# agustinus/emqx

Hardware: AMD Instinct MI355X
Metric: publishes matched/sec (node) at 1M wildcard subs; p99 batch match latency (higher is better)
Workload: dtype u32; 1 GPU; C2: 1M wildcard filters depth<=7, 10M-publish batch per GPU; filters=1000000, publishes_per_gpu=10000000, mode=replicated, parallelism=replicated trie x1, batches split per GPU, batches_in_flight=1

## Files before the change

emqx_amd/csrc/tm_kernels.hip:

```cpp
#include <algorithm>
#include <cstddef>
#include <cstdlib>
#include "tm_internal.hpp"

namespace etm {

constexpr int TILE = 64;
constexpr int WCAP = 512;
#ifndef TM_WPE384
#define TM_WPE384 4
#endif

constexpr uint32_t M_LVL_SHIFT = 6;
constexpr uint32_t M_LVL_MASK = 0xF;
constexpr uint32_t M_PLUS = 1u << 10;
constexpr uint32_t M_SKIPE = 1u << 11;
constexpr uint32_t M_DSTART = 1u << 12;
static_assert(FAST_MAX_DEPTH <= (int)M_LVL_MASK, "level field too narrow");
constexpr uint32_t M_DISP_SHIFT = 13;
constexpr uint32_t M_DISP_MASK = 0x3F;
static_assert(MAX_PROBE_DISP <= M_DISP_MASK, "the displacement field holds every bounded probe run");
constexpr uint32_t Q_FOUND = ~((1u << LSIG_BITS) - 1u);
constexpr uint32_t Q_TAIL = 0xFFFFFFFFu;

__device__ __forceinline__ uint32_t dig_L(uint32_t c) { return (0x4432u >> (4 * c)) & 0xF; }
__device__ __forceinline__ uint32_t dig_H(uint32_t c) { return (0x2223u >> (4 * c)) & 0xF; }
__device__ __forceinline__ uint32_t dig_P(uint32_t c) { return (0x3344u >> (4 * c)) & 0xF; }

__device__ __forceinline__ int key_shift(uint32_t level) { return 61 - 3 * (int)level; }

__device__ __forceinline__ uint64_t put_digit(uint64_t key, uint32_t level, uint32_t d) {
    return level <= FAST_MAX_DEPTH ? (key | ((uint64_t)d << key_shift(level))) : key;
}

__device__ __forceinline__ uint32_t prefix_count(uint64_t mask) {
    return __builtin_amdgcn_mbcnt_hi((uint32_t)(mask >> 32), __builtin_amdgcn_mbcnt_lo((uint32_t)mask, 0u));
}

template <bool CK>
__device__ __forceinline__ uint64_t ck(uint64_t i, uint64_t bound, uint32_t* dbg, uint32_t id) {
    if (CK && i >= bound) {
        if (dbg) {
            if (atomicCAS(&dbg[0], 0u, id) == 0u) { dbg[1] = (uint32_t)i; dbg[2] = (uint32_t)bound; }
            atomicAdd(&dbg[3], 1u);
        }
        return 0;
    }
    return i;
}
#define CK_(i, bound, id) ck<CK>((i), (bound), a.dbg, (id))

struct Node {
    uint32_t child;
    uint32_t term;
    uint32_t hterm;
    uint32_t flags;
};

#ifndef TM_PROBE_CPOL
#define TM_PROBE_CPOL 0
#endif
__device__ __forceinline__ uint4 ld_b128(__amdgpu_buffer_rsrc_t r, uint32_t off) {
    const auto v = __builtin_amdgcn_raw_buffer_load_b128(r, (int)off, 0, TM_PROBE_CPOL);
    return uint4{v[0], v[1], v[2], v[3]};
}

template <bool CK, bool BIG>
__device__ __forceinline__ bool probe(const MatchArgs& a, uint32_t parent, uint32_t word, Node& n) {
    uint32_t b = home_bucket(parent, word, a.nbuckets);
    const bool small = !BIG;
    const __amdgpu_buffer_rsrc_t rs = __builtin_amdgcn_make_buffer_rsrc(
        const_cast<Slot*>(a.slots), 0, BIG ? 0u : a.nslots * 16u, 0x00020000);
    for (uint32_t p = 0; p <= a.max_probe; ++p) {
        uint4 s0, s1, s2, s3;
        const uint64_t si = CK_((uint64_t)b * BUCKET, a.nslots, 1);
        if (small) {
            const uint32_t off = (uint32_t)si * 16u;
            s0 = ld_b128(rs, off); s1 = ld_b128(rs, off + 16); s2 = ld_b128(rs, off + 32); s3 = ld_b128(rs, off + 48);
        } else {
            const uint4* q = reinterpret_cast<const uint4*>(a.slots) + si;
            s0 = q[0]; s1 = q[1]; s2 = q[2]; s3 = q[3];
        }
        const bool m0 = (s0.x & ID_MASK) == parent && (s0.y & WID_MASK) == word;
        const bool m1 = (s1.x & ID_MASK) == parent && (s1.y & WID_MASK) == word;
        const bool m2 = (s2.x & ID_MASK) == parent && (s2.y & WID_MASK) == word;
        const bool m3 = (s3.x & ID_MASK) == parent && (s3.y & WID_MASK) == word;
        const uint32_t hz = m0 ? s0.z : m1 ? s1.z : m2 ? s2.z : s3.z;
        const uint32_t hw = m0 ? s0.w : m1 ? s1.w : m2 ? s2.w : s3.w;
        if (m0 | m1 | m2 | m3) {
            n.child = hz & ID_MASK;
            n.term = (hz & B_TOPIC) ? n.child : NONE;
            n.hterm = (hw & B_HTERM) ? (hw & ID_MASK) : NONE;
            n.flags = ((hz & B_PLUS) ? NF_PLUS : 0u) | ((hw & B_HASH) ? NF_HASH : 0u);
            return true;
        }
        if (s3.x == SLOT_EMPTY) return false;
        b = (b + 1 == a.nbuckets) ? 0 : b + 1;
    }
    return false;
}

struct Expand {
    uint32_t ne, np;
    uint32_t ef0, ef1;
    uint64_t ek0, ek1;
    uint32_t pf0, pf1;
    uint64_t pk0, pk1;
};

__device__ __forceinline__ void add_e(Expand& x, uint32_t fid, uint64_t key) {
    if (x.ne == 0) { x.ef0 = fid; x.ek0 = key; } else { x.ef1 = fid; x.ek1 = key; }
    x.ne++;
}
__device__ __forceinline__ void add_p(Expand& x, uint64_t key, uint32_t fl) {
    if (x.np == 0) { x.pk0 = key; x.pf0 = fl; } else { x.pk1 = key; x.pf1 = fl; }
    x.np++;
}

__device__ __forceinline__ void expand(const Node& s, uint32_t lc, uint32_t d, uint32_t flags,
                                       uint64_t key, uint32_t w_here, uint32_t w_prev, Expand& x) {
    x.ne = 0; x.np = 0;
    if (lc == d) {
        if (!(flags & M_SKIPE) && s.term != NONE) {
            uint64_t k = key;
            if ((w_prev >> WID_BITS) == C_EMPTY && lc - 1 <= FAST_MAX_DEPTH) {
                const int sp = key_shift(lc - 1);
                if (((k >> sp) & 7) == 4) k = (k & ~(7ull << sp)) | (1ull << sp);
            }
            add_e(x, s.term, k);
        }
        if (s.hterm != NONE) add_e(x, s.hterm, put_digit(key, lc, 2));
        return;
    }
    const uint32_t cls = w_here >> WID_BITS, id = w_here & WID_MASK;
    if (s.hterm != NONE) add_e(x, s.hterm, put_digit(key, lc, dig_H(cls)));
    if (id == W_HASH) {
        if (s.flags & NF_HASH) add_p(x, put_digit(key, lc, dig_L(cls)), (lc + 1 == d) ? M_SKIPE : 0u);
    } else if (id != W_UNKNOWN && id != W_PLUS) {
        add_p(x, put_digit(key, lc, dig_L(cls)), 0u);
    }
    if (s.flags & NF_PLUS) add_p(x, put_digit(key, lc, dig_P(cls)), M_PLUS);
}

__device__ __forceinline__ void expand_root(const RootRec& r, bool dollar, uint32_t d, uint32_t w0, Expand& x) {
    x.ne = 0; x.np = 0;
    const uint32_t cls = w0 >> WID_BITS, id = w0 & WID_MASK;
    if (!dollar && r.hterm != NONE) add_e(x, r.hterm, (uint64_t)dig_H(cls) << 61);
    if (id == W_HASH) {
        if (!dollar && (r.flags & NF_HASH)) add_p(x, (uint64_t)dig_L(cls) << 61, (d == 1) ? M_SKIPE : 0u);
    } else if (id != W_UNKNOWN && id != W_PLUS) {
        add_p(x, (uint64_t)dig_L(cls) << 61, dollar ? M_DSTART : 0u);
    }
    if (!dollar && (r.flags & NF_PLUS)) add_p(x, (uint64_t)dig_P(cls) << 61, M_PLUS);
}

template <int QC>
struct alignas(16) TileLds {
    static constexpr int QCAP = QC;
    uint4 q[QC];
    uint32_t words[WCAP];
    uint32_t toff[TILE];
    uint32_t depth[TILE];
    uint32_t cnt[TILE];
    uint32_t list[TILE];
    static constexpr uint32_t STAGE = (QC * 16 + WCAP * 4) / 8;
};

__device__ __forceinline__ uint4 q_pack(uint64_t key, uint32_t meta, uint32_t parent, uint32_t pw) {
    return uint4{(uint32_t)key | meta, (uint32_t)(key >> 32), parent, pw};
}

static_assert(offsetof(TileLds<512>, words) + sizeof(uint32_t) * WCAP == TileLds<512>::STAGE * 8,
              "staging area must be contiguous");
static_assert(offsetof(TileLds<384>, words) + sizeof(uint32_t) * WCAP == TileLds<384>::STAGE * 8,
              "staging area must be contiguous");

__device__ __forceinline__ uint32_t xor_lane32(uint32_t v, uint32_t j) {
    const uint32_t lane = threadIdx.x & 63;
    switch (j) {
    case 1: return (uint32_t)__builtin_amdgcn_mov_dpp((int)v, 0xB1, 0xF, 0xF, false);
    case 2: return (uint32_t)__builtin_amdgcn_mov_dpp((int)v, 0x4E, 0xF, 0xF, false);
    case 4: return (uint32_t)__builtin_amdgcn_mov_dpp(__builtin_amdgcn_mov_dpp((int)v, 0x141, 0xF, 0xF, false), 0x1B, 0xF,
                                                      0xF, false);
    case 8: return (uint32_t)__builtin_amdgcn_mov_dpp((int)v, 0x128, 0xF, 0xF, false);
    case 16: {
        const auto p = __builtin_amdgcn_permlane16_swap(v, v, false, false);
        return (lane & 16) ? p[0] : p[1];
    }
    default: {
        const auto p = __builtin_amdgcn_permlane32_swap(v, v, false, false);
        return (lane & 32) ? p[0] : p[1];
    }
    }
}

__device__ __forceinline__ unsigned long long xor_lane64(unsigned long long v, uint32_t j) {
    return ((unsigned long long)xor_lane32((uint32_t)(v >> 32), j) << 32) | xor_lane32((uint32_t)v, j);
}

__device__ __forceinline__ uint32_t tile_sum(uint32_t v) {
#pragma unroll
    for (uint32_t j = 1; j < 64; j <<= 1) v += xor_lane32(v, j);
    return __builtin_amdgcn_readfirstlane(v);
}

enum : int { PH_PROLOGUE = 0, PH_LOOP = 1, PH_READBACK = 2, PH_SORT = 3 };
struct PhaseClk {
#if TM_PHASE_CYCLES
    unsigned long long sum[PHASE_N] = {0, 0, 0, 0}, t0 = 0;
    __device__ __forceinline__ void start() { t0 = __builtin_readcyclecounter(); }
    __device__ __forceinline__ void lap(int p) {
        const unsigned long long now = __builtin_readcyclecounter();
        sum[p] += now - t0;
        t0 = now;
    }
#else
    __device__ __forceinline__ void start() {}
    __device__ __forceinline__ void lap(int) {}
#endif
};

__device__ __forceinline__ uint32_t xor_lane32_bc(uint32_t v, uint32_t j) {
    const int x = (int)v;
    switch (j) {
    case 1: return (uint32_t)__builtin_amdgcn_update_dpp(0, x, 0xB1, 0xF, 0xF, true);
    case 2: return (uint32_t)__builtin_amdgcn_update_dpp(0, x, 0x4E, 0xF, 0xF, true);
    case 4: return (uint32_t)__builtin_amdgcn_update_dpp(0, __builtin_amdgcn_update_dpp(0, x, 0x141, 0xF, 0xF, true),
                                                         0x1B, 0xF, 0xF, true);
    default: return (uint32_t)__builtin_amdgcn_update_dpp(0, x, 0x128, 0xF, 0xF, true);
    }
}

#ifndef TM_TAGGED_SORT
#define TM_TAGGED_SORT 1
#endif
constexpr uint64_t keep_lo_mask(uint32_t W, uint32_t kk, uint32_t j) {
    uint64_t m = 0;
    for (uint32_t l = 0; l < 64; ++l) {
        const uint32_t e = l & (W - 1);
        if (((e & j) == 0) == ((e & kk) == 0)) m |= 1ull << l;
    }
    return m;
}

template <uint32_t W, uint32_t KK, uint32_t J>
__device__ __forceinline__ uint32_t tag_stage(uint32_t k) {
    constexpr uint64_t M = keep_lo_mask(W, KK, J);
    uint32_t lo, hi;
    if constexpr (J >= 16) {
        const auto p = J == 16 ? __builtin_amdgcn_permlane16_swap(k, k, false, false)
                               : __builtin_amdgcn_permlane32_swap(k, k, false, false);
        lo = min(p[0], p[1]);
        hi = max(p[0], p[1]);
    } else {
        const uint32_t other = xor_lane32_bc(k, J);
        lo = min(k, other);
        hi = max(k, other);
    }
    return __builtin_amdgcn_inverse_ballot_w64(M) ? lo : hi;
}
template <uint32_t W, uint32_t KK, uint32_t J>
__device__ __forceinline__ uint32_t tag_merge(uint32_t k) {
    k = tag_stage<W, KK, J>(k);
    if constexpr (J > 1) k = tag_merge<W, KK, J / 2>(k);
    return k;
}
template <uint32_t W, uint32_t KK = 2>
__device__ __forceinline__ uint32_t tag_sort(uint32_t k) {
    k = tag_merge<W, KK, KK / 2>(k);
    if constexpr (KK < W) k = tag_sort<W, KK * 2>(k);
    return k;
}

template <bool CK, class LT>
__device__ __forceinline__ void sort_classes(const MatchArgs& a, LT& L, bool keep, uint32_t c, uint32_t pos,
                                             uint32_t dst, uint32_t free) {
    constexpr uint32_t STAGE = LT::STAGE;
    const uint32_t lane = threadIdx.x;
    const unsigned long long* stg = reinterpret_cast<const unsigned long long*>(L.q);
    if (keep && c == 1) a.sfids[CK_(dst, a.sfids_cap, 40)] = (uint32_t)(stg[CK_(pos, STAGE, 41)] & ~KEY_MASK);
#pragma unroll
    for (uint32_t W = 2; W <= 64; W <<= 1) {
        const bool mine = keep && c > W / 2 && c <= W;
        const uint64_t m = __ballot(mine);
        if (!m) continue;
        const uint32_t nrows = __popcll(m);
        if (mine) L.list[prefix_count(m)] = lane;
        __syncthreads();
        const uint32_t e = lane & (W - 1);
        const uint32_t STEP = 64 / W;
        for (uint32_t g = 0; g < nrows; g += STEP) {
            const uint32_t r = g + lane / W;
            const bool rv = r < nrows;
            const uint32_t owner = rv ? L.list[r] : 0u;
            const uint32_t cr = __shfl(c, owner, 64);
            const uint32_t pr = __shfl(pos, owner, 64);
            const uint32_t dr = __shfl(dst, owner, 64);
            if (TM_TAGGED_SORT && (W >> free) <= 1) {
                const uint32_t* stg32 = reinterpret_cast<const uint32_t*>(L.q);
                uint32_t k32 = 0xFFFFFFFFu;
                if (rv && e < cr) k32 = stg32[2 * CK_(pr + e, STAGE, 42) + 1] | e;
                switch (W) {
                case 2: k32 = tag_sort<2>(k32); break;
                case 4: k32 = tag_sort<4>(k32); break;
                case 8: k32 = tag_sort<8>(k32); break;
                case 16: k32 = tag_sort<16>(k32); break;
                case 32: k32 = tag_sort<32>(k32); break;
                default: k32 = tag_sort<64>(k32); break;
                }
                if (rv && e < cr)
                    a.sfids[CK_((uint64_t)dr + e, a.sfids_cap, 44)] =
                        stg32[2 * CK_(pr + (k32 & (W - 1)), STAGE, 43)] & (uint32_t)~KEY_MASK;
                continue;
            }
            unsigned long long key = ~0ull;
            if (rv && e < cr) key = stg[CK_(pr + e, STAGE, 42)];
#pragma unroll
            for (uint32_t kk = 2; kk <= W; kk <<= 1) {
#pragma unroll
                for (uint32_t j = kk >> 1; j > 0; j >>= 1) {
                    const unsigned long long other = xor_lane64(key, j);
                    const bool up = (e & kk) == 0;
                    const bool lower = (e & j) == 0;
                    const unsigned long long lo = key < other ? key : other;
                    const unsigned long long hi = key < other ? other : key;
                    key = (lower == up) ? lo : hi;
                }
            }
            if (rv && e < cr) a.sfids[CK_((uint64_t)dr + e, a.sfids_cap, 44)] = (uint32_t)(key & ~KEY_MASK);
        }
        __syncthreads();
    }
    {
        const bool mine = keep && c > 64;
        uint64_t m = __ballot(mine);
        while (m) {
            const uint32_t owner = (uint32_t)__builtin_ctzll(m);
            m &= m - 1;
            const uint32_t cr = __shfl(c, owner, 64);
            const uint32_t pr = __shfl(pos, owner, 64);
            const uint32_t dr = __shfl(dst, owner, 64);
            unsigned long long k0 = ~0ull, k1 = ~0ull;
            if (lane < cr) k0 = stg[CK_(pr + lane, STAGE, 45)];
            if (lane + 64 < cr) k1 = stg[CK_(pr + lane + 64, STAGE, 46)];
            uint32_t r0 = 0, r1 = 0;
            for (uint32_t j = 0; j < 64; ++j) {
                const unsigned long long kj = __shfl(k0, j, 64);
                r0 += kj < k0 ? 1u : 0u;
                r1 += kj < k1 ? 1u : 0u;
            }
            for (uint32_t j = 64; j < cr; ++j) {
                const unsigned long long kj = __shfl(k1, j - 64, 64);
                r0 += kj < k0 ? 1u : 0u;
                r1 += kj < k1 ? 1u : 0u;
            }
            if (lane < cr) a.sfids[CK_((uint64_t)dr + r0, a.sfids_cap, 47)] = (uint32_t)(k0 & ~KEY_MASK);
            if (lane + 64 < cr) a.sfids[CK_((uint64_t)dr + r1, a.sfids_cap, 48)] = (uint32_t)(k1 & ~KEY_MASK);
        }
    }
}

#ifndef TM_PREFETCH_NEXT
#define TM_PREFETCH_NEXT 2
#endif
struct TileAhead {
    uint32_t off, end, fl;
#if TM_PREFETCH_NEXT >= 2
    uint32_t w[WCAP / 64];
#endif
};

template <bool CK>
__device__ __forceinline__ void ahead_meta(const MatchArgs& a, uint32_t tile, uint32_t tt, TileAhead& p) {
    const uint32_t lane = threadIdx.x;
    const uint32_t t = tile * tt + lane;
    p.off = 0; p.end = 0; p.fl = TF_SLOW;
    if (lane < tt && t < a.n) {
        p.off = a.toff[CK_(t, a.n + 1, 4)];
        p.end = a.toff[CK_(t + 1, a.n + 1, 5)];
        p.fl = a.tflags[CK_(t, a.n, 6)];
    }
}

__device__ __forceinline__ void ahead_range(const MatchArgs& a, uint32_t tile, uint32_t tt, const TileAhead& p,
                                            uint32_t& wbeg, uint32_t& wend) {
    const uint32_t nv = min(tt, a.n - tile * tt);
    wbeg = __builtin_amdgcn_readlane(p.off, 0);
    wend = __builtin_amdgcn_readlane(p.end, nv - 1);
}

template <bool CK>
__device__ __forceinline__ void ahead_words(const MatchArgs& a, uint32_t tile, uint32_t tt, TileAhead& p) {
#if TM_PREFETCH_NEXT >= 2
    const uint32_t lane = threadIdx.x;
    uint32_t wbeg, wend;
    ahead_range(a, tile, tt, p, wbeg, wend);
    const uint32_t nw = wend - wbeg;
    if (nw > (uint32_t)WCAP) return;
#pragma unroll
    for (uint32_t j = 0; j < WCAP / 64; ++j) {
        const uint32_t i = lane + 64 * j;
        if (i < nw) p.w[j] = a.words[CK_(wbeg + i, a.nwords, 8)];
    }
#endif
}

#ifndef TM_LOG_U
#define TM_LOG_U 12
#endif
template <bool CK, class LT, class AW>
__device__ __forceinline__ void sort_rows_log(const MatchArgs& a, LT& L, bool keep, uint32_t c, uint32_t dst,
                                              unsigned long long* wlog, uint8_t* wlane, uint32_t lcount,
                                              PhaseClk& pc, const AW& ah_words) {
    constexpr uint32_t STAGE = LT::STAGE;
    const uint32_t lane = threadIdx.x;
    unsigned long long* stg = reinterpret_cast<unsigned long long*>(L.q);
    const uint32_t cw = keep ? c : 0u;
    uint32_t incl = cw;
    for (int o = 1; o < 64; o <<= 1) {
        const uint32_t u = __shfl_up(incl, o, 64);
        if (lane >= (uint32_t)o) incl += u;
    }
    const uint32_t pos = incl - cw;
    uint32_t rs = 0;
    while (rs < a.tile_topics) {
        const uint32_t p0 = __builtin_amdgcn_readlane(pos, rs);
        const uint64_t beyond = __ballot(lane >= rs && pos + cw - p0 > STAGE);
        const uint32_t re = beyond ? (uint32_t)__builtin_ctzll(beyond) : a.tile_topics;
        const bool in_chunk = keep && lane >= rs && lane < re;
        L.depth[lane] = in_chunk ? pos - p0 : NONE;
        L.toff[lane] = 0;
        __syncthreads();
        uint32_t kor = 0;
        for (uint32_t k0 = 0; k0 < lcount; k0 += 64 * TM_LOG_U) {
            unsigned long long e[TM_LOG_U];
            uint32_t r[TM_LOG_U];
#pragma unroll
            for (uint32_t u = 0; u < TM_LOG_U; ++u) {
                const uint32_t k = k0 + lane + 64 * u;
                r[u] = 64;
                if (k < lcount) {
                    e[u] = wlog[k];
                    r[u] = wlane[k];
                }
            }
#pragma unroll
            for (uint32_t u = 0; u < TM_LOG_U; ++u) {
                const uint32_t base = r[u] < 64 ? L.depth[r[u]] : NONE;
                if (base == NONE) continue;
                const uint32_t at = base + atomicAdd(&L.toff[r[u]], 1u);
                stg[CK_(at, STAGE, 49)] = e[u];
                kor |= (uint32_t)(e[u] >> 31);
            }
        }
        uint32_t free = 0;
        if (TM_TAGGED_SORT) {
#pragma unroll
            for (uint32_t j = 1; j < 64; j <<= 1) kor |= xor_lane32(kor, j);
            const uint32_t tz = (uint32_t)__builtin_ctz(__builtin_amdgcn_readfirstlane(kor) | 0x200u);
            free = tz ? tz - 1 : 0u;
        }
        __syncthreads();
        pc.lap(PH_READBACK);
        if (rs == 0) ah_words();
        sort_classes<CK, LT>(a, L, in_chunk, c, pos - p0, dst, free);
        __syncthreads();
        pc.lap(PH_SORT);
        rs = re;
    }
}

template <bool CK>
__device__ __forceinline__ void send_to_slow(const MatchArgs& a, bool mine, uint32_t t) {
    const uint64_t m = __ballot(mine);
    uint32_t base = 0;
    if (threadIdx.x == 0 && m) base = atomicAdd(&a.ctrl[CTRL_NOVF], (uint32_t)__popcll(m));
    base = __shfl(base, 0, 64);
    if (mine) {
        const uint32_t slot = base + prefix_count(m);
        if (slot < a.ovf_cap) a.ovf_list[CK_(slot, a.ovf_cap, 12)] = t;
        else atomicOr(&a.ctrl[CTRL_ERR], ERR_OVF_LIST);
    }
}

template <bool CK, bool BIG, bool IN_LDS, class LT, class AM, class AW>
__device__ __forceinline__ void match_tile(const MatchArgs& a, LT& L, uint32_t t0, uint32_t tend, uint32_t wbase,
                                           uint8_t fl, bool valid, unsigned long long& sV, unsigned long long& sH,
                                           unsigned long long& sW, unsigned long long& sM, unsigned long long& sP,
                                           PhaseClk& pc, const AM& ah_meta, const AW& ah_words) {
    const uint32_t lane = threadIdx.x;
    const uint32_t t = t0 + lane;
    const uint32_t* wsrc = IN_LDS ? L.words : a.words;
    const uint32_t wlim = IN_LDS ? (uint32_t)WCAP : a.nwords;
    (void)wbase;

    uint32_t qn = 0;
    const bool active = !(fl & TF_SLOW);
    unsigned long long* const wrows = a.rows + (uint64_t)blockIdx.x * a.tile_topics * a.row_cap;
    const uint32_t lcap = a.tile_topics * a.row_cap;
    uint8_t* const wlane =
        reinterpret_cast<uint8_t*>(a.rows + (uint64_t)a.grid * lcap) + (uint64_t)blockIdx.x * lcap;
    uint32_t lcount = 0;
    uint32_t tV = 0, tH = 0, tP = 0;
    const uint32_t d_me = L.depth[lane];

    {
        Expand x; x.ne = 0; x.np = 0;
        uint32_t w0 = 0;
        if (active && d_me > 0) {
            const bool dollar = fl & TF_DOLLAR;
            tV += 1;
            if (!dollar && (a.root.flags & NF_HASH)) tH += 1;
            w0 = wsrc[CK_(L.toff[lane], wlim, 9)];
            expand_root(a.root, dollar, d_me, w0, x);
        }
        const uint64_t b0 = __ballot(x.np >= 1), b1 = __ballot(x.np >= 2);
        const uint32_t pre = prefix_count(b0) + prefix_count(b1);
        const uint32_t meta = lane | (1u << M_LVL_SHIFT);
        const uint32_t wid = w0 & WID_MASK;
        if (x.np >= 1) L.q[qn + pre] = q_pack(x.pk0, meta | x.pf0, ROOT, (x.pf0 & M_PLUS) ? W_PLUS : wid);
        if (x.np >= 2) L.q[qn + pre + 1] = q_pack(x.pk1, meta | x.pf1, ROOT, (x.pf1 & M_PLUS) ? W_PLUS : wid);
        qn += __popcll(b0) + __popcll(b1);
        const uint64_t mr = __ballot(x.ne != 0);
        if (x.ne) {
            L.cnt[lane] = 1;
            const uint32_t i = prefix_count(mr);
            wrows[i] = (x.ek0 & KEY_MASK) | x.ef0;
            wlane[i] = (uint8_t)lane;
        }
        lcount = (uint32_t)__popcll(mr);
    }

    const uint32_t qd = lane >> 2, qs = lane & 3;
    uint32_t nbk = a.nbuckets, maxp = a.max_probe, rcap = a.row_cap, nrec = BIG ? 0u : a.nslots * 16u;
    Slot* sbase = const_cast<Slot*>(a.slots);
    asm volatile("" : "+s"(nbk), "+s"(maxp), "+s"(rcap), "+s"(nrec), "+s"(sbase));
    uint64_t wbits = IN_LDS ? 0ull : (uint64_t)a.words;
    if constexpr (!IN_LDS) asm volatile("" : "+s"(wbits));
    typedef const __attribute__((address_space(1))) uint32_t* gwords_t;
    typedef uint32_t u32x4_t __attribute__((ext_vector_type(4)));
    typedef const __attribute__((address_space(1))) u32x4_t* gslots_t;
    const auto word_at = [&](uint64_t i) -> uint32_t { return IN_LDS ? L.words[i] : ((gwords_t)wbits)[i]; };
    pc.lap(PH_PROLOGUE);
    while (qn > 0) {
        const uint32_t k = min(qn, 64u);
        const bool has = lane < k;
        qn -= k;
        tP += k + (1u << 20);
        asm volatile("" : "+v"(tP));
        const uint32_t idx = qn + (has ? lane : 0u);
        const uint4 e = L.q[idx];
        const uint32_t meta = e.x & 0x7FFFFFFFu;
        const uint64_t key = ((uint64_t)e.y << 32) | (e.x & 0x80000000u);
        const uint32_t parent = e.z, pw = e.w;
        const uint32_t tl = meta & 63;
        const uint32_t lc = (meta >> M_LVL_SHIFT) & M_LVL_MASK;
        const uint32_t disp = (meta >> M_DISP_SHIFT) & M_DISP_MASK;
        {
            uint32_t hb = home_bucket(parent, pw, nbk) + disp;
            if (hb >= nbk) hb -= nbk;
            L.q[idx].x = hb;
        }
        asm volatile("" : "+s"(sbase), "+s"(nrec));
        const __amdgpu_buffer_rsrc_t rsrc = __builtin_amdgcn_make_buffer_rsrc(sbase, 0, nrec, 0x00020000);
        uint32_t rp[4], rw[4];
        uint4 sl[4];
#pragma unroll
        for (uint32_t r = 0; r < 4; ++r) {
            const uint32_t p = 16 * r + qd;
            const bool v = p < k;
            const uint4 rec = L.q[qn + (v ? p : 0u)];
            rp[r] = v ? rec.z : SLOT_EMPTY;
            rw[r] = rec.w;
            const uint64_t si = CK_((uint64_t)rec.x * BUCKET + qs, a.nslots, 1);
            if (!BIG) {
                sl[r] = ld_b128(rsrc, v ? (uint32_t)si * 16u : 0xFFFFFFF0u);
            } else {
                const u32x4_t g = v ? ((gslots_t)(uint64_t)sbase)[si] : u32x4_t{0u, 0u, 0u, 0u};
                sl[r] = uint4{g[0], g[1], g[2], g[3]};
            }
        }
        __builtin_amdgcn_sched_barrier(0);
        const uint32_t base = L.toff[tl];
        const uint32_t d = L.depth[tl];
        const bool at_end = lc == d;
        const uint32_t w_here = word_at(CK_(base + lc - (at_end ? 1u : 0u), wlim, 11));
        const uint32_t w_prev = word_at(CK_(base + lc - 1, wlim, 10));
#pragma unroll
        for (uint32_t r = 0; r < 4; ++r) {
            const bool m = (sl[r].x & ID_MASK) == rp[r] && (sl[r].y & WID_MASK) == rw[r];
            if (m) {
                L.q[qn + 16 * r + qd].x = sl[r].z;
                L.q[qn + 16 * r + qd].y = sl[r].w;
                L.q[qn + 16 * r + qd].z = Q_FOUND | slot_lsig(sl[r].x, sl[r].y);
            }
        }
        uint32_t qs_now = qs;
        asm volatile("" : "+v"(qs_now));
        if (qs_now == 3) {
#pragma unroll
            for (uint32_t r = 0; r < 4; ++r) L.q[qn + 16 * r + qd].w = sl[r].x == SLOT_EMPTY ? Q_TAIL : rw[r];
        }
        const uint4 res = L.q[idx];
        const bool live = has & (L.cnt[tl] <= rcap);
        const bool found = live & (res.z >= Q_FOUND);
        const bool cont = live & !found & (res.w != Q_TAIL) & (disp < maxp);
        const uint32_t hz = res.x, hw = res.y;
        const uint32_t child = hz & ID_MASK, hterm = hw & ID_MASK;
        const bool n_topic = (hz & B_TOPIC) != 0, n_plus = (hz & B_PLUS) != 0;
        const bool n_hterm = (hw & B_HTERM) != 0, n_hash = (hw & B_HASH) != 0;
        const uint32_t cls = w_here >> WID_BITS, id = w_here & WID_MASK;
        const int sh = key_shift(lc);
        tV += (found & !(meta & M_DSTART)) ? 1u : 0u;
        tH += (found & n_hash) ? 1u : 0u;
        const bool eA0 = found & (at_end ? (!(meta & M_SKIPE) & n_topic) : n_hterm);
        const bool eB0 = found & at_end & n_hterm;
        const uint32_t fA = at_end ? child : hterm;
        const int sp = sh + 3;
        const bool redigit = ((w_prev >> WID_BITS) == C_EMPTY) & (((key >> sp) & 7) == 4);
        const uint64_t kA = key ^ ((uint64_t)(at_end ? (redigit ? 5u : 0u) : dig_H(cls)) << (at_end ? sp : sh));
        const bool lit = (id != W_UNKNOWN) & (id != W_PLUS) & (((res.z >> lsig_pos(id)) & 1u) != 0) &
                         (n_hash | (((hw >> lext_pos(id)) & 1u) != 0));
        const bool pL = found & !at_end & (id == W_HASH ? n_hash : lit);
        const bool pP = found & !at_end & n_plus;
        bool eA = eA0, eB = eB0;
        const bool sL = cont | pL;
        const uint64_t bL = __ballot(sL), bP = __ballot(pP);
        const uint32_t ptot = __popcll(bL) + __popcll(bP);
        if (qn + ptot > (uint32_t)LT::QCAP) break;
        const uint32_t pre = qn + prefix_count(bL) + prefix_count(bP);
        const uint32_t nmeta = tl | ((lc + 1) << M_LVL_SHIFT);
        if (sL) {
            const uint32_t lfl = ((id == W_HASH) & (lc + 1 == d)) ? M_SKIPE : 0u;
            const uint64_t kL = cont ? key : key | ((uint64_t)dig_L(cls) << sh);
            L.q[pre] = q_pack(kL, cont ? meta + (1u << M_DISP_SHIFT) : nmeta | lfl, cont ? parent : child,
                              cont ? pw : id);
        }
        if (pP) L.q[pre + (sL ? 1u : 0u)] = q_pack(key | ((uint64_t)dig_P(cls) << sh), nmeta | M_PLUS, child, W_PLUS);
        qn += ptot;
        {
            uint32_t slot = 0;
            if (eA | eB) slot = atomicAdd(&L.cnt[tl], (eA ? 1u : 0u) + (eB ? 1u : 0u));
            const uint32_t slotB = slot + (eA ? 1u : 0u);
            eA = eA && slot < rcap;
            eB = eB && slotB < rcap;
            const uint64_t mA = __ballot(eA), mB = __ballot(eB);
            const uint32_t nA = (uint32_t)__popcll(mA), nE = nA + (uint32_t)__popcll(mB);
            if (eA) {
                const uint32_t i = lcount + prefix_count(mA);
                wrows[CK_(i, lcap, 13)] = (kA & KEY_MASK) | fA;
                wlane[i] = (uint8_t)tl;
            }
            if (eB) {
                const uint32_t i = lcount + nA + prefix_count(mB);
                wrows[CK_(i, lcap, 14)] = ((key | (2ull << sh)) & KEY_MASK) | hterm;
                wlane[i] = (uint8_t)tl;
            }
            lcount += nE;
        }
    }
    __syncthreads();
    pc.lap(PH_LOOP);
    ah_meta();

    if (qn > 0) {
        send_to_slow<CK>(a, valid && active, t);
        ah_words();
        return;
    }
    sV += tile_sum(tV); sH += tile_sum(tH);
    sW += tile_sum((active && L.depth[lane] > 0) ? L.depth[lane] : 0u);
    {
        const uint32_t p = __builtin_amdgcn_readfirstlane(tP);
        sP += (p & 0xFFFFFu) | ((unsigned long long)(p >> 20) << 40);
    }
    const uint32_t c_me = L.cnt[lane];
    const bool row_ovf = valid && active && c_me > a.row_cap;
    send_to_slow<CK>(a, row_ovf, t);
    const bool keep = valid && active && !row_ovf;
    const uint32_t c = keep ? c_me : 0u;
    uint32_t incl = c;
    for (int o = 1; o < 64; o <<= 1) {
        const uint32_t u = __shfl_up(incl, o, 64);
        if (lane >= (uint32_t)o) incl += u;
    }
    const uint32_t tot = __shfl(incl, 63, 64);
    unsigned long long base64 = 0;
    const uint32_t g = (blockIdx.x % TICKET_GROUPS) & a.sgmask;
    if (lane == 0 && tot) base64 = atomicAdd(xg_top(a.xg, g), (unsigned long long)tot);
    base64 = __shfl(base64, 0, 64);
    const bool fits = base64 + tot <= a.rcap;
    base64 += (uint64_t)g * a.rcap;
    const uint32_t base = (uint32_t)base64;
    const uint32_t dst = base + incl - c;
    pc.lap(PH_SORT);
    if (fits) {
        sort_rows_log<CK, LT>(a, L, keep, c, dst, wrows, wlane, lcount, pc, ah_words);
    } else {
        if (lane == 0) atomicOr(&a.ctrl[CTRL_ERR], ERR_STAGING);
        ah_words();
    }
    if (keep) {
        a.count[CK_(t, a.n, 16)] = c_me;
        a.src[CK_(t, a.n, 17)] = dst;
    }
    sM += __builtin_amdgcn_readfirstlane(tot);
    pc.lap(PH_SORT);
    (void)tend;
}

#ifndef TM_DN_TILES_PER_WAVE
#define TM_DN_TILES_PER_WAVE 4
#endif
constexpr uint32_t DN_TILES_PER_WAVE = TM_DN_TILES_PER_WAVE;

template <bool CK, bool BIG, int QC>
__global__ __launch_bounds__(64) __attribute__((amdgpu_waves_per_eu(QC == 384 ? TM_WPE384 : 3, 8))) void tm_match_tiles(MatchArgs a) {
    __shared__ TileLds<QC> L;
    if (a.d_n) {
        a.n = *a.d_n;
        while (a.tile_topics > 1 && (a.n + a.tile_topics - 1) / a.tile_topics < DN_TILES_PER_WAVE * gridDim.x)
            a.tile_topics >>= 1;
        const uint32_t nt = (a.n + a.tile_topics - 1) / a.tile_topics;
        a.static_rounds = max(1u, nt / (2u * gridDim.x));
    }
    const uint32_t lane = threadIdx.x;
    const uint32_t tt = a.tile_topics;
    const uint32_t ntiles = (a.n + tt - 1) / tt;
    unsigned long long sV = 0, sH = 0, sW = 0, sM = 0, sP = 0;
    PhaseClk pc;

    uint32_t tile = blockIdx.x, round = 0;
#if TM_PREFETCH_NEXT
    TileAhead nx;
    if (tile < ntiles) {
        ahead_meta<CK>(a, tile, tt, nx);
        ahead_words<CK>(a, tile, tt, nx);
    }
#endif
    while (tile < ntiles) {
        pc.start();
        uint32_t ticket = 0;
        if (round + 1 >= a.static_rounds && lane == 0)
            ticket = atomicAdd(&a.xg[(blockIdx.x % TICKET_GROUPS) * TICKET_STRIDE], 1u);
        const uint32_t t0 = tile * tt;
        const uint32_t tend = min(t0 + tt, a.n);
        const uint32_t t = t0 + lane;
        const bool valid = lane < tt && t < a.n;
#if TM_PREFETCH_NEXT
        uint32_t wbeg, wend;
        ahead_range(a, tile, tt, nx, wbeg, wend);
        const bool in_lds = (wend - wbeg) <= (uint32_t)WCAP;
        const uint32_t my_off = valid ? nx.off : wend;
        const uint32_t my_end = valid ? nx.end : wend;
        const uint8_t fl = (uint8_t)nx.fl;
#if TM_PREFETCH_NEXT >= 2
        if (in_lds) {
#pragma unroll
            for (uint32_t j = 0; j < WCAP / 64; ++j) {
                const uint32_t i = lane + 64 * j;
                if (i < wend - wbeg) L.words[CK_(i, WCAP, 7)] = nx.w[j];
            }
        }
#else
        if (in_lds)
            for (uint32_t i = lane; i < wend - wbeg; i += 64) L.words[CK_(i, WCAP, 7)] = a.words[CK_(wbeg + i, a.nwords, 8)];
#endif
#else
        const uint32_t wbeg = a.toff[CK_(t0, a.n + 1, 2)], wend = a.toff[CK_(tend, a.n + 1, 3)];
        const bool in_lds = (wend - wbeg) <= (uint32_t)WCAP;
        const uint32_t my_off = valid ? a.toff[CK_(t, a.n + 1, 4)] : wend;
        const uint32_t my_end = valid ? a.toff[CK_(t + 1, a.n + 1, 5)] : wend;
        const uint8_t fl = valid ? a.tflags[CK_(t, a.n, 6)] : (uint8_t)TF_SLOW;
        if (in_lds)
// ... 2745 lines not shown
            slow = (fl & TF_SLOW) != 0;
            out.w0 = w0;
            out.nw = tn;
            out.fl = fl;
        }
        tok_append_slow(a, slow, t);
        __syncthreads();
    } else {
        const uint64_t o = tile_base + tincl - nw;
        if (valid) {
            a.toff[t] = (uint32_t)o;
            out.fl = tok_fill_topic_global(a, t, o, slow);
            out.w0 = tincl - nw;
            out.nw = nw;
        }
        tok_append_slow(a, slow, t);
    }
}

#ifndef TM_TOK_WPE
#define TM_TOK_WPE 5
#endif
__global__ __launch_bounds__(64) __attribute__((amdgpu_waves_per_eu(TM_TOK_WPE, 8))) void tm_tok_fill(TokArgs a) {
    __shared__ TokLds L;
    if (a.d_n) a.n = *a.d_n;
    const uint32_t tt = a.tile_topics;
    const uint32_t ntiles = (a.n + tt - 1) / tt;
    TokTile out;
    for (uint32_t tile = blockIdx.x; tile < ntiles; tile += gridDim.x) tok_tile<TOK_WPL_FILL>(a, L, tile, nullptr, out);
}


__global__ __launch_bounds__(256) void tm_export_host(ExportArgs a) {
    const uint64_t stride = (uint64_t)gridDim.x * 256;
    const uint64_t i0 = (uint64_t)blockIdx.x * 256 + threadIdx.x;
    if (a.d_n) {
        a.n = *a.d_n;
        a.hdr_words = a.fixed_words + 2 * a.n;
        a.h_count = a.h_hdr + a.hdr_words;
    }
    for (uint64_t i = i0; i < a.hdr_words; i += stride) a.h_hdr[i] = a.hdr[i];
    for (uint64_t i = i0; i < a.n; i += stride) a.h_count[i] = a.count[i];
    for (uint32_t g = 0; g < TICKET_GROUPS; ++g) {
        const uint64_t top = xg_top_read(a.hdr, g);
        const uint64_t lo = g * a.rcap, hi = lo + (top < a.rcap ? top : a.rcap);
        for (uint64_t i = lo + i0; i < hi && i < a.rows_cap; i += stride) a.h_rows[i] = a.rows[i];
    }
}

__global__ __launch_bounds__(256) void tm_csr_to_host(const uint32_t* row_off, const uint32_t* ids, uint32_t n,
                                                       const uint32_t* d_total, uint64_t cap, uint32_t* h_row,
                                                       uint32_t* h_ids) {
    const uint64_t stride = (uint64_t)gridDim.x * 256;
    const uint64_t i0 = (uint64_t)blockIdx.x * 256 + threadIdx.x;
    const uint64_t total = min((uint64_t)*d_total, cap);
    for (uint64_t i = i0; i <= n; i += stride) h_row[i] = row_off[i];
    for (uint64_t i = i0; i < total; i += stride) h_ids[i] = ids[i];
}

hipError_t launch_csr_to_host(const uint32_t* row_off, const uint32_t* ids, uint32_t n, const uint32_t* d_total,
                              uint64_t cap, uint32_t* h_row, uint32_t* h_ids, hipStream_t s) {
    const uint64_t work = std::max<uint64_t>(cap, (uint64_t)n + 1);
    const uint32_t grid = (uint32_t)std::min<uint64_t>(std::max<uint64_t>((work / 8 + 255) / 256, 1), 1024);
    hipLaunchKernelGGL(tm_csr_to_host, dim3(grid), dim3(256), 0, s, row_off, ids, n, d_total, cap, h_row, h_ids);
    return hipGetLastError();
}

__global__ __launch_bounds__(256) void tm_pack_ids(const uint32_t* ids, uint64_t n, uint8_t* out) {
    const uint64_t g = (uint64_t)blockIdx.x * 256 + threadIdx.x, j = 4 * g;
    if (j >= n) return;
    if (j + 4 <= n) {
        const uint4 v = *reinterpret_cast<const uint4*>(ids + j);
        uint32_t* o = reinterpret_cast<uint32_t*>(out + 12 * g);
        o[0] = (v.x & 0xFFFFFFu) | (v.y << 24);
        o[1] = ((v.y >> 8) & 0xFFFFu) | (v.z << 16);
        o[2] = ((v.z >> 16) & 0xFFu) | (v.w << 8);
        return;
    }
    for (uint64_t q = j; q < n; ++q)
        for (uint32_t b = 0; b < 3; ++b) out[3 * q + b] = (uint8_t)(ids[q] >> (8 * b));
}

hipError_t launch_pack_ids(const uint32_t* ids, uint64_t n, uint8_t* out, hipStream_t s) {
    const uint64_t groups = (n + 3) / 4;
    if (groups) hipLaunchKernelGGL(tm_pack_ids, dim3((uint32_t)((groups + 255) / 256)), dim3(256), 0, s, ids, n, out);
    return hipGetLastError();
}

hipError_t launch_export_host(const ExportArgs& a, hipStream_t s) {
    const uint64_t work = a.hdr_words + a.n + a.rows_cap;
    const uint32_t grid = (uint32_t)std::min<uint64_t>(std::max<uint64_t>((work / 4 + 255) / 256, 1), 512);
    hipLaunchKernelGGL(tm_export_host, dim3(grid), dim3(256), 0, s, a);
    return hipGetLastError();
}

__global__ void tm_scatter_keys(DictKey* keys, const uint32_t* idx, const DictKey* vals, uint32_t n) {
    const uint32_t i = blockIdx.x * blockDim.x + threadIdx.x;
    if (i < n) keys[idx[i]] = vals[i];
}


#ifndef TM_MIN_TILES
#define TM_MIN_TILES 256
#endif
uint32_t tile_topics(uint32_t n) {
    uint32_t tt = 64;
    while (tt > 1 && (n + tt - 1) / tt < TM_MIN_TILES) tt >>= 1;
    return tt;
}

uint32_t match_waves(uint32_t n, int device, uint32_t qcap) {
    static uint32_t cap[64][2] = {};
    const int qi = qcap <= 384 ? 0 : 1;
    const uint32_t tt = tile_topics(n);
    const uint32_t ntiles = (n + tt - 1) / tt;
    uint32_t c = (device >= 0 && device < 64) ? cap[device][qi] : 0u;
    if (!c) {
        int per_cu = 0, cus = 0;
        if (hipOccupancyMaxActiveBlocksPerMultiprocessor(
                &per_cu, qi == 0 ? tm_match_tiles<false, false, 384> : tm_match_tiles<false, false, 512>, 64, 0) !=
                hipSuccess ||
            hipDeviceGetAttribute(&cus, hipDeviceAttributeMultiprocessorCount, device) != hipSuccess ||
            per_cu <= 0 || cus <= 0) {
            (void)hipGetLastError();
            per_cu = qi == 0 ? 16 : 14;
            cus = 256;
        }
        if (const char* w = getenv("TM_WAVES_PER_CU")) per_cu = std::min(per_cu, std::max(1, atoi(w)));
        c = (uint32_t)per_cu * (uint32_t)cus;
        if (device >= 0 && device < 64) cap[device][qi] = c;
    }
    return ntiles < c ? ntiles : c;
}

template <bool CK, bool BIG>
static hipError_t launch_match_t(const MatchArgs& a, hipStream_t s, hipEvent_t ev_a, hipEvent_t ev_b,
                                 unsigned ev_flags) {
    const uint32_t ntiles = (a.n + a.tile_topics - 1) / a.tile_topics;
    hipError_t e;
    if (ev_a && (e = hipEventRecordWithFlags(ev_a, s, ev_flags)) != hipSuccess) return e;
    if (ntiles) {
        const uint32_t grid = a.grid;
        if (a.qcap <= 384) hipLaunchKernelGGL((tm_match_tiles<CK, BIG, 384>), dim3(grid), dim3(64), 0, s, a);
        else hipLaunchKernelGGL((tm_match_tiles<CK, BIG, 512>), dim3(grid), dim3(64), 0, s, a);
    }
    if (ev_b && (e = hipEventRecordWithFlags(ev_b, s, ev_flags)) != hipSuccess) return e;
    if (ntiles && a.wstats) hipLaunchKernelGGL(tm_stats_reduce, dim3(1), dim3(256), 0, s, a.wstats, a.grid, a.stats);
    hipLaunchKernelGGL((tm_match_slow<CK, BIG>), dim3(a.s_waves), dim3(64), 0, s, a);
    return hipSuccess;
}

hipError_t launch_match(const MatchArgs& a, hipStream_t s, hipEvent_t ev_a, hipEvent_t ev_b, bool checked,
                        unsigned ev_flags) {
    const bool big = (uint64_t)a.nslots * sizeof(Slot) > 0xFFFFFFFFull;
    hipError_t e;
    if (checked) e = big ? launch_match_t<true, true>(a, s, ev_a, ev_b, ev_flags)
                         : launch_match_t<true, false>(a, s, ev_a, ev_b, ev_flags);
    else e = big ? launch_match_t<false, true>(a, s, ev_a, ev_b, ev_flags)
                 : launch_match_t<false, false>(a, s, ev_a, ev_b, ev_flags);
    if (e != hipSuccess) return e;
    return hipGetLastError();
}

hipError_t launch_scan(const ScanArgs& a, hipStream_t s, uint32_t* d_total) {
    const uint32_t nb = scan_block_count(a.n);
    if (nb <= 1) {
        hipLaunchKernelGGL(tm_scan_local, dim3(1), dim3(SCAN_BLOCK), 0, s, a, d_total);
        return hipGetLastError();
    }
    hipLaunchKernelGGL(tm_scan_local, dim3(nb), dim3(SCAN_BLOCK), 0, s, a, (uint32_t*)nullptr);
    hipLaunchKernelGGL(tm_scan_sums, dim3(1), dim3(SCAN_BLOCK), 0, s, a, nb, d_total);
    return hipGetLastError();
}

hipError_t launch_finalize(const ScanArgs& a, hipStream_t s, bool checked) {
    const uint32_t ntiles = (a.n + TILE - 1) / TILE;
    if (!ntiles) return hipGetLastError();
    const uint32_t grid = min(ntiles, 256u * 32u);
    if (checked) hipLaunchKernelGGL(tm_finalize<true>, dim3(grid), dim3(64), 0, s, a);
    else hipLaunchKernelGGL(tm_finalize<false>, dim3(grid), dim3(64), 0, s, a);
    return hipGetLastError();
}

hipError_t launch_shared_count(const SharedArgs& a, hipStream_t s) {
    if (a.m) hipLaunchKernelGGL(tm_shared_count, dim3((a.m + 255) / 256), dim3(256), 0, s, a);
    return hipGetLastError();
}

hipError_t launch_shared_rows(const SharedArgs& a, hipStream_t s) {
    hipLaunchKernelGGL(tm_shared_rows, dim3((a.n + 1 + 255) / 256), dim3(256), 0, s, a);
    return hipGetLastError();
}

hipError_t launch_shared_pick(const SharedArgs& a, hipStream_t s) {
    if (a.m) hipLaunchKernelGGL(tm_shared_pick, dim3((a.m + 255) / 256), dim3(256), 0, s, a);
    return hipGetLastError();
}

hipError_t launch_shared_fold(SharedSlot* slots, const uint2* upd, uint32_t nslots, hipStream_t s) {
    if (nslots) hipLaunchKernelGGL(tm_shared_fold, dim3((nslots + 255) / 256), dim3(256), 0, s, slots, upd, nslots);
    return hipGetLastError();
}

hipError_t launch_route_count(const RouteArgs& a, hipStream_t s) {
    if (a.m) hipLaunchKernelGGL(tm_route_count, dim3((a.m + 255) / 256), dim3(256), 0, s, a);
    return hipGetLastError();
}

hipError_t launch_route_rows(const RouteArgs& a, hipStream_t s) {
    hipLaunchKernelGGL(tm_route_rows, dim3((a.n + 1 + 255) / 256), dim3(256), 0, s, a);
    return hipGetLastError();
}

hipError_t launch_route_fill(const RouteArgs& a, hipStream_t s) {
    if (a.m) hipLaunchKernelGGL(tm_route_fill, dim3((a.m + 255) / 256), dim3(256), 0, s, a);
    return hipGetLastError();
}

hipError_t launch_fan_scan(const FanArgs& a, hipStream_t s) {
    const uint64_t ne = a.n_matches + 1;
    const uint32_t nb = (uint32_t)((ne + FAN_SCAN_TILE - 1) / FAN_SCAN_TILE);
    hipLaunchKernelGGL(tm_fan_scan_local, dim3(nb), dim3(FAN_BLOCK), 0, s, a);
    hipLaunchKernelGGL(tm_fan_scan_sums, dim3(1), dim3(FAN_BLOCK), 0, s, a, nb);
    if (a.nreg) {
        if (a.n) hipLaunchKernelGGL(tm_fan_rows_stg, dim3((a.n + FAN_BLOCK - 1) / FAN_BLOCK), dim3(FAN_BLOCK), 0, s, a);
    } else {
        hipLaunchKernelGGL(tm_fan_rows, dim3((a.n + 1 + FAN_BLOCK - 1) / FAN_BLOCK), dim3(FAN_BLOCK), 0, s, a);
    }
    return hipGetLastError();
}

hipError_t launch_fan_globalize(const FanArgs& a, hipStream_t s) {
    const uint64_t ne = a.n_matches + 1;
    hipLaunchKernelGGL(tm_fan_scan_add, dim3((uint32_t)((ne + FAN_BLOCK - 1) / FAN_BLOCK)), dim3(FAN_BLOCK), 0, s, a);
    return hipGetLastError();
}

hipError_t launch_fan_fill(const FanArgs& a, hipStream_t s) {
    if (a.total) {
        const uint64_t nt = (a.total + FAN_FILL_TILE - 1) / FAN_FILL_TILE;
        hipLaunchKernelGGL(tm_fan_tiles, dim3((uint32_t)((nt + 1 + FAN_BLOCK - 1) / FAN_BLOCK)), dim3(FAN_BLOCK), 0, s,
                           a, nt);
        if (a.out_j) {
            if (a.total > a.big_limit) hipLaunchKernelGGL((tm_fan_fill<true, true>), dim3((uint32_t)nt), dim3(FAN_BLOCK), 0, s, a);
            else hipLaunchKernelGGL((tm_fan_fill<false, true>), dim3((uint32_t)nt), dim3(FAN_BLOCK), 0, s, a);
        } else if (a.total > a.big_limit) hipLaunchKernelGGL(tm_fan_fill<true>, dim3((uint32_t)nt), dim3(FAN_BLOCK), 0, s, a);
        else hipLaunchKernelGGL(tm_fan_fill<false>, dim3((uint32_t)nt), dim3(FAN_BLOCK), 0, s, a);
    }
    return hipGetLastError();
}

hipError_t launch_inbox_pubof(const InboxArgs& a, hipStream_t s) {
    if (a.m && a.n) hipLaunchKernelGGL(tm_inbox_pubof, dim3((a.m + 255) / 256), dim3(256), 0, s, a);
    return hipGetLastError();
}

hipError_t launch_inbox_sort(const InboxArgs& a, hipStream_t s) {
    if (!a.D || !a.ntiles || a.passes > INBOX_MAX_PASSES) return hipGetLastError();
    ScanArgs sa{};
    sa.count = a.hist; sa.row_off = a.hist; sa.block_sums = a.hbs; sa.n = 256u * a.ntiles;
    for (uint32_t p = 0; p < a.passes; ++p) {
        const uint32_t* kin = p & 1 ? a.key1 : a.key0;
        const uint32_t* vin = p & 1 ? a.val1 : a.val0;
        uint32_t* kout = p & 1 ? a.key0 : a.key1;
        uint32_t* vout = p & 1 ? a.val0 : a.val1;
        hipLaunchKernelGGL(tm_inbox_hist, dim3(a.ntiles), dim3(INBOX_BLOCK), 0, s, a, kin, a.hist, 8 * p);
        const hipError_t e = launch_scan(sa, s, nullptr);
        if (e != hipSuccess) return e;
        hipLaunchKernelGGL(tm_inbox_scatter, dim3(a.ntiles), dim3(INBOX_BLOCK), 0, s, a, kin, vin, kout, vout,
                           (const uint32_t*)a.hist, (const uint32_t*)a.hbs, 8 * p);
    }
    return hipGetLastError();
}

hipError_t launch_inbox_merge(const MergeArgs& a, hipStream_t s) {
    const uint64_t tot = (uint64_t)a.nd + a.ns;
    if (tot) hipLaunchKernelGGL(tm_inbox_merge, dim3((uint32_t)((tot + 255) / 256)), dim3(256), 0, s, a);
    return hipGetLastError();
}

hipError_t launch_inbox_finish(const InboxArgs& a, hipStream_t s) {
    if (!a.D || !a.ntiles) return hipGetLastError();
    const uint32_t* keys = a.passes & 1 ? a.key1 : a.key0;
    const uint32_t* vals = a.passes & 1 ? a.val1 : a.val0;
    if (a.mrec) hipLaunchKernelGGL(tm_inbox_finish<true>, dim3(a.ntiles), dim3(INBOX_BLOCK), 0, s, a, keys, vals);
    else hipLaunchKernelGGL(tm_inbox_finish<false>, dim3(a.ntiles), dim3(INBOX_BLOCK), 0, s, a, keys, vals);
    ScanArgs sa{};
    sa.count = a.hcount; sa.row_off = a.hcount; sa.block_sums = a.hcbs; sa.n = a.ntiles;
    const hipError_t e = launch_scan(sa, s, a.d_R);
    if (e != hipSuccess) return e;
    hipLaunchKernelGGL(tm_inbox_heads, dim3(a.ntiles), dim3(INBOX_BLOCK), 0, s, a, keys);
    return hipGetLastError();
}

hipError_t launch_deliver_flags(const DeliverArgs& a, bool drop, hipStream_t s) {
    if (!a.D || !a.R || !a.ntiles) return hipGetLastError();
    hipLaunchKernelGGL(tm_deliver_range, dim3((a.R + 255) / 256), dim3(256), 0, s, a);
    if (a.groups) {
        if (drop)
            hipLaunchKernelGGL((tm_deliver_flags<true, true>), dim3(a.ntiles), dim3(INBOX_BLOCK), 0, s, a);
        else
            hipLaunchKernelGGL((tm_deliver_flags<false, true>), dim3(a.ntiles), dim3(INBOX_BLOCK), 0, s, a);
    } else if (drop)
        hipLaunchKernelGGL((tm_deliver_flags<true, false>), dim3(a.ntiles), dim3(INBOX_BLOCK), 0, s, a);
    else
        hipLaunchKernelGGL((tm_deliver_flags<false, false>), dim3(a.ntiles), dim3(INBOX_BLOCK), 0, s, a);
    return hipGetLastError();
// ... 197 lines not shown
```

Measured before the change: 2.562 billion publishes/s.

## Map each quad to four consecutive queue entries and broadcast probe inputs via DPP

```diff
diff --git a/emqx_amd/csrc/tm_kernels.hip b/emqx_amd/csrc/tm_kernels.hip
--- a/emqx_amd/csrc/tm_kernels.hip
+++ b/emqx_amd/csrc/tm_kernels.hip
@@ -20,8 +20,14 @@
 constexpr uint32_t M_DISP_SHIFT = 13;
 constexpr uint32_t M_DISP_MASK = 0x3F;
 static_assert(MAX_PROBE_DISP <= M_DISP_MASK, "the displacement field holds every bounded probe run");
+#ifndef TM_QUAD_OWN
+#define TM_QUAD_OWN 1
+#endif
+#if TM_QUAD_OWN != 1
 constexpr uint32_t Q_FOUND = ~((1u << LSIG_BITS) - 1u);
 constexpr uint32_t Q_TAIL = 0xFFFFFFFFu;
+#endif
+constexpr uint32_t OFF_NONE = 0xFFFFFFC0u;
 
 __device__ __forceinline__ uint32_t dig_L(uint32_t c) { return (0x4432u >> (4 * c)) & 0xF; }
 __device__ __forceinline__ uint32_t dig_H(uint32_t c) { return (0x2223u >> (4 * c)) & 0xF; }
@@ -228,6 +234,16 @@
     case 4: return (uint32_t)__builtin_amdgcn_update_dpp(0, __builtin_amdgcn_update_dpp(0, x, 0x141, 0xF, 0xF, true),
                                                          0x1B, 0xF, 0xF, true);
     default: return (uint32_t)__builtin_amdgcn_update_dpp(0, x, 0x128, 0xF, 0xF, true);
+    }
+}
+
+__device__ __forceinline__ uint32_t quad_bcast(uint32_t v, uint32_t r) {
+    const int x = (int)v;
+    switch (r) {
+    case 0: return (uint32_t)__builtin_amdgcn_update_dpp(0, x, 0x00, 0xF, 0xF, true);
+    case 1: return (uint32_t)__builtin_amdgcn_update_dpp(0, x, 0x55, 0xF, 0xF, true);
+    case 2: return (uint32_t)__builtin_amdgcn_update_dpp(0, x, 0xAA, 0xF, 0xF, true);
+    default: return (uint32_t)__builtin_amdgcn_update_dpp(0, x, 0xFF, 0xF, 0xF, true);
     }
 }
 
@@ -532,6 +548,7 @@
     }
 
     const uint32_t qd = lane >> 2, qs = lane & 3;
+    const auto q_of = [&](uint32_t r) -> uint32_t { return TM_QUAD_OWN ? 4 * qd + r : 16 * r + qd; };
     uint32_t nbk = a.nbuckets, maxp = a.max_probe, rcap = a.row_cap, nrec = BIG ? 0u : a.nslots * 16u;
     Slot* sbase = const_cast<Slot*>(a.slots);
     asm volatile("" : "+s"(nbk), "+s"(maxp), "+s"(rcap), "+s"(nrec), "+s"(sbase));
@@ -556,18 +573,33 @@
         const uint32_t tl = meta & 63;
         const uint32_t lc = (meta >> M_LVL_SHIFT) & M_LVL_MASK;
         const uint32_t disp = (meta >> M_DISP_SHIFT) & M_DISP_MASK;
-        {
-            uint32_t hb = home_bucket(parent, pw, nbk) + disp;
-            if (hb >= nbk) hb -= nbk;
-            L.q[idx].x = hb;
-        }
+        uint32_t hb = home_bucket(parent, pw, nbk) + disp;
+        if (hb >= nbk) hb -= nbk;
+#if TM_QUAD_OWN
+        if (CK) hb = (uint32_t)(CK_((uint64_t)hb * BUCKET + (BUCKET - 1), a.nslots, 1) / BUCKET);
+        const uint32_t o_par = has ? parent : SLOT_EMPTY;
+        const uint32_t o_bkt = BIG ? (has ? hb : 0u) : (has ? hb * (uint32_t)(BUCKET * sizeof(Slot)) : OFF_NONE);
+#else
+        L.q[idx].x = hb;
+#endif
         asm volatile("" : "+s"(sbase), "+s"(nrec));
         const __amdgpu_buffer_rsrc_t rsrc = __builtin_amdgcn_make_buffer_rsrc(sbase, 0, nrec, 0x00020000);
         uint32_t rp[4], rw[4];
         uint4 sl[4];
 #pragma unroll
         for (uint32_t r = 0; r < 4; ++r) {
-            const uint32_t p = 16 * r + qd;
+#if TM_QUAD_OWN
+            rp[r] = quad_bcast(o_par, r);
+            rw[r] = quad_bcast(pw, r);
+            const uint32_t ob = quad_bcast(o_bkt, r);
+            if (!BIG) {
+                sl[r] = ld_b128(rsrc, ob + qs * (uint32_t)sizeof(Slot));
+            } else {
+                const u32x4_t g = ((gslots_t)(uint64_t)sbase)[(uint64_t)ob * BUCKET + qs];
+                sl[r] = uint4{g[0], g[1], g[2], g[3]};
+            }
+#else
+            const uint32_t p = q_of(r);
             const bool v = p < k;
             const uint4 rec = L.q[qn + (v ? p : 0u)];
             rp[r] = v ? rec.z : SLOT_EMPTY;
@@ -579,6 +611,7 @@
                 const u32x4_t g = v ? ((gslots_t)(uint64_t)sbase)[si] : u32x4_t{0u, 0u, 0u, 0u};
                 sl[r] = uint4{g[0], g[1], g[2], g[3]};
             }
+#endif
         }
         __builtin_amdgcn_sched_barrier(0);
         const uint32_t base = L.toff[tl];
@@ -586,26 +619,45 @@
         const bool at_end = lc == d;
         const uint32_t w_here = word_at(CK_(base + lc - (at_end ? 1u : 0u), wlim, 11));
         const uint32_t w_prev = word_at(CK_(base + lc - 1, wlim, 10));
+        uint32_t qs_now = qs;
+        asm volatile("" : "+v"(qs_now));
+#if TM_QUAD_OWN == 1
+        if (qs_now == 3) {
+#pragma unroll
+            for (uint32_t r = 0; r < 4; ++r) L.q[qn + q_of(r)].w = sl[r].x;
+        }
+#pragma unroll
+        for (uint32_t r = 0; r < 4; ++r) {
+            const bool m = (sl[r].x & ID_MASK) == rp[r] && (sl[r].y & WID_MASK) == rw[r];
+            if (m) L.q[qn + q_of(r)] = sl[r];
+        }
+        const uint4 res = L.q[idx];
+        const bool live = has & (L.cnt[tl] <= rcap);
+        const bool found = live & (res.z != parent);
+        const bool cont = live & !found & (res.w != SLOT_EMPTY) & (disp < maxp);
+        const uint32_t hz = res.z, hw = res.w;
+        const uint32_t lsig = slot_lsig(res.x, res.y);
+#else
 #pragma unroll
         for (uint32_t r = 0; r < 4; ++r) {
             const bool m = (sl[r].x & ID_MASK) == rp[r] && (sl[r].y & WID_MASK) == rw[r];
             if (m) {
-                L.q[qn + 16 * r + qd].x = sl[r].z;
-                L.q[qn + 16 * r + qd].y = sl[r].w;
-                L.q[qn + 16 * r + qd].z = Q_FOUND | slot_lsig(sl[r].x, sl[r].y);
-            }
-        }
-        uint32_t qs_now = qs;
-        asm volatile("" : "+v"(qs_now));
+                L.q[qn + q_of(r)].x = sl[r].z;
+                L.q[qn + q_of(r)].y = sl[r].w;
+                L.q[qn + q_of(r)].z = Q_FOUND | slot_lsig(sl[r].x, sl[r].y);
+            }
+        }
         if (qs_now == 3) {
 #pragma unroll
-            for (uint32_t r = 0; r < 4; ++r) L.q[qn + 16 * r + qd].w = sl[r].x == SLOT_EMPTY ? Q_TAIL : rw[r];
+            for (uint32_t r = 0; r < 4; ++r) L.q[qn + q_of(r)].w = sl[r].x == SLOT_EMPTY ? Q_TAIL : rw[r];
         }
         const uint4 res = L.q[idx];
         const bool live = has & (L.cnt[tl] <= rcap);
         const bool found = live & (res.z >= Q_FOUND);
         const bool cont = live & !found & (res.w != Q_TAIL) & (disp < maxp);
         const uint32_t hz = res.x, hw = res.y;
+        const uint32_t lsig = res.z;
+#endif
         const uint32_t child = hz & ID_MASK, hterm = hw & ID_MASK;
         const bool n_topic = (hz & B_TOPIC) != 0, n_plus = (hz & B_PLUS) != 0;
         const bool n_hterm = (hw & B_HTERM) != 0, n_hash = (hw & B_HASH) != 0;
@@ -619,7 +671,7 @@
         const int sp = sh + 3;
         const bool redigit = ((w_prev >> WID_BITS) == C_EMPTY) & (((key >> sp) & 7) == 4);
         const uint64_t kA = key ^ ((uint64_t)(at_end ? (redigit ? 5u : 0u) : dig_H(cls)) << (at_end ? sp : sh));
-        const bool lit = (id != W_UNKNOWN) & (id != W_PLUS) & (((res.z >> lsig_pos(id)) & 1u) != 0) &
+        const bool lit = (id != W_UNKNOWN) & (id != W_PLUS) & (((lsig >> lsig_pos(id)) & 1u) != 0) &
                          (n_hash | (((hw >> lext_pos(id)) & 1u) != 0));
         const bool pL = found & !at_end & (id == W_HASH ? n_hash : lit);
         const bool pP = found & !at_end & n_plus;
@@ -3671,7 +3723,7 @@
 
 hipError_t launch_match(const MatchArgs& a, hipStream_t s, hipEvent_t ev_a, hipEvent_t ev_b, bool checked,
                         unsigned ev_flags) {
-    const bool big = (uint64_t)a.nslots * sizeof(Slot) > 0xFFFFFFFFull;
+    const bool big = (uint64_t)a.nslots * sizeof(Slot) > (uint64_t)OFF_NONE;
     hipError_t e;
     if (checked) e = big ? launch_match_t<true, true>(a, s, ev_a, ev_b, ev_flags)
                          : launch_match_t<true, false>(a, s, ev_a, ev_b, ev_flags);
```

Result: faster. 2.655 billion publishes/s (median of 6 runs) (+3.6%).
